# NivekNey/polars-matmul

Measured on AMD Instinct MI355X. Metric: cosine top-k queries/sec, higher is better.
Workload: dtype f32

## Files before the change

polars-matmul_amd/csrc/pmm_capi.hip:

```cpp
#include "pmm_internal.h"
#include "../../include/pmm.h"

#include <hip/hip_runtime.h>

#include <algorithm>
#include <atomic>
#include <cmath>
#include <cstdarg>
#include <cstdio>
#include <cstdlib>
#include <cstring>
#include <mutex>
#include <string>
#include <type_traits>
#include <vector>

using namespace pmm;

namespace {

constexpr const char *kVersion = "0.1.4+mi355x.r1";
constexpr size_t kMaterialiseBudget = size_t(2) << 30;

thread_local std::string t_err;
// ... 877 lines not shown
                               out_score, s));
  return PMM_OK;
}

int topk_f32_screened(const TopkRoute &r, const float *q, int64_t ldq, int64_t m, const float *c, int64_t ldc,
                      int64_t n, int64_t d, int64_t k, uint32_t index_base, uint32_t *out_idx, float *out_score,
                      char *w, hipStream_t s, int cus, const ScreenImage *img = nullptr,
                      const float *c_norms = nullptr) {
  const int metric = kMetricCosine;
  const ScreenPlan &sp = r.sp;
  const Plan &p = r.p;
  float *qn = (float *)(w + p.off_qn);
  const float *cn = img ? c_norms : (float *)(w + p.off_cn);
  uint16_t *qb = (uint16_t *)(w + sp.off_qb);
  const uint16_t *cb = img ? img->cb : (uint16_t *)(w + sp.off_cb);
  float *rel = (float *)(w + sp.off_rel), *eps = (float *)(w + sp.off_eps);
  unsigned *bad = (unsigned *)(w + sp.off_bad), *ovf = (unsigned *)(w + sp.off_ovf);
  unsigned *scal = (unsigned *)(w + sp.off_scal);
  int *rows = (int *)(w + sp.off_rows);
  HIP_TRY(hipMemsetAsync(w, 0, p.off_gthr + (size_t)m * 8, s));
  if (p.qb_full) HIP_TRY(hipMemsetAsync(w + p.off_cnt, 0, (size_t)m * p.S * 4, s));
  HIP_TRY(hipMemsetAsync(w + sp.off_ovf, 0, sp.off_rows - sp.off_ovf, s));
  if (img) {
    Timed t("norms_f32/prepare", s);
    HIP_TRY(launch_screen_prepare(q, m, d, ldq, qb, sp.dpb, qn, nullptr, rel, bad, nullptr, s));
    uint32_t bits;
    memcpy(&bits, &img->max_rel, 4);
    HIP_TRY(hipMemsetD32Async((hipDeviceptr_t)scal, (int)bits, 1, s));
  } else {
    Timed t("norms_f32/round", s);
    float *wcn = (float *)(w + p.off_cn), *crel = (float *)(w + sp.off_crel);
    HIP_TRY(launch_screen_prepare(q, m, d, ldq, qb, sp.dpb, qn, nullptr, rel, bad, nullptr, s));
    HIP_TRY(launch_screen_prepare(c, n, d, ldc, (uint16_t *)(w + sp.off_cb), sp.dpb, wcn, wcn + n, crel,
                                  (unsigned *)(crel + n), scal, s));
  }
  GemmF32Args a = fused_args(m, n, sp.dpb, k, metric, p, w);
  a.qb = qb;
  a.cb = cb;
  a.qn = qn;
  a.cn = cn;
  a.cpre = cn + n;
  a.ldq = sp.dpb;
  a.ldc = sp.dpb;
  set_bf16_knobs(a);
  const bool debug = getenv("PMM_SCREEN_DEBUG") != nullptr;
  a.eps = eps;
  a.ovf = ovf;
  {
    const int64_t ns = kSeedMaxNs;
    const int seed_env = getenv("PMM_BF16_SEED") ? atoi(getenv("PMM_BF16_SEED")) : 1;
    const bool seeded = seed_env && 4 * k <= ns && n >= 8 * ns && (size_t)m * ns * 4 <= p.off_qn - p.off_cand;
    Timed t("seed_bf16/screen", s);
    if (seeded) {
      float *sample = (float *)a.cand;
      HIP_TRY(launch_seed_bf16_ws(a, sample, (int)ns, s));
      HIP_TRY(launch_seed_select(sample, ns, (int)m, (int)ns, (int)k, metric, a.gthr, s));
    }
    HIP_TRY(launch_screen_prep(rel, scal, (int)m, (int)sp.dpb, eps, a.gthr, seeded ? 1 : 0, s));
  }
  {
    Timed t("gemm_f32_topk/screen", s);
    HIP_TRY(launch_gemm_bf16_ws(a, p.grid, s, true));
  }
  {
    Timed t("merge_topk/rescore", s);
    ScreenFinishArgs fa{};
    fa.q = q;
    fa.c = c;
    fa.ldq = ldq;
    fa.ldc = ldc;
    fa.qn = qn;
    fa.cn = cn;
    fa.eps = eps;
    fa.M = (int)m;
    fa.N = (int)n;
    fa.dp = (int)sp.dp;
    fa.S = p.S;
    fa.capg = p.capg;
    fa.k = (int)k;
    fa.cand = a.cand;
    fa.cnt = a.cnt;
    fa.gthr = a.gthr;
    fa.stat = debug ? scal + 4 : nullptr;
    HIP_TRY(launch_screen_rescore(fa, s));
  }
  {
    Timed t("merge_topk", s);
    HIP_TRY(launch_merge(merge_cand_args(a, p, index_base, out_idx, out_score), 0, s));
  }
  HIP_TRY(launch_zero_sign_f32(q, ldq, c, ldc, qn, cn, (int)m, n, (int)d, (int)k, metric, index_base, out_idx,
                               out_score, s));
  HIP_TRY(launch_screen_collect(ovf, bad, (int)m, scal + 2, rows, s));
  unsigned h[8] = {0, 0, 0, 0, 0, 0, 0, 0};
  HIP_TRY(hipMemcpyAsync(h, scal, 32, hipMemcpyDeviceToHost, s));
  HIP_TRY(hipStreamSynchronize(s));
  const bool whole = h[1] != 0 || (int64_t)h[2] * 8 > m + 8 * kScreenRerunRows;
  if (debug) {
    float rc;
    memcpy(&rc, &h[0], 4);
    fprintf(stderr,
            "[pmm screen] S=%d tps=%d qb_full=%d capg=%d ctrig=%d corpus_residual=%.6g corpus_unsafe=%u "
            "rerun_rows=%u overflowed=%u whole_call_f32=%d rescored=%u max_per_row=%u kept=%u m=%lld handle=%d\n",
            p.S, p.tps, p.qb_full, p.capg, p.ctrig, rc, h[1], h[2], h[3], whole ? 1 : 0, h[4], h[5], h[6],
            (long long)m, img ? 1 : 0);
  }
  if (whole) {
    const TopkRoute f = route_topk(m, n, d, k, metric, PMM_COMPUTE_F32, cus, false, false);
    return topk_f32_fused(f.p, q, ldq, m, c, ldc, n, d, k, metric, index_base, out_idx, out_score, w + sp.off_f32,
                          s, cus, c_norms, false);
  }
  for (int64_t r0 = 0; r0 < (int64_t)h[2]; r0 += sp.rr) {
    const int64_t nr = std::min<int64_t>(sp.rr, (int64_t)h[2] - r0);
    const TopkRoute f = route_topk(nr, n, d, k, metric, PMM_COMPUTE_F32, cus, false, false);
    const int rc = rerun_rows(q, ldq * 4, sp.dp * 4, rows + r0, nr, k, f.total, w + sp.off_gq, sp.total - sp.off_gq,
                              out_idx, out_score, s, "screen re-run",
                              [&](const char *gq, uint32_t *gi, float *gs, char *fw) {
                                return topk_f32_fused(f.p, (const float *)gq, sp.dp, nr, c, ldc, n, d, k, metric,
                                                      index_base, gi, gs, fw, s, cus, c_norms, false);
                              });
    if (rc) return rc;
  }
  return PMM_OK;
}

int topk_f32_unscreened(const TopkRoute &r, const float *q, int64_t ldq, int64_t m, const float *c, int64_t ldc,
                        int64_t n, int64_t d, int64_t k, int metric, uint32_t index_base, uint32_t *out_idx,
                        float *out_score, char *w, hipStream_t s, int cus, const float *c_norms, bool keep_gthr,
                        const float *c_pre = nullptr) {
  return r.fused ? topk_f32_fused(r.p, q, ldq, m, c, ldc, n, d, k, metric, index_base, out_idx, out_score, w, s, cus,
                                  c_norms, keep_gthr, c_pre)
                 : topk_f32_materialised(r.mp, q, ldq, m, c, ldc, n, d, k, metric, index_base, out_idx, out_score, w,
                                         s, cus, c_norms);
}

int topk_f32_device_impl(const TopkRoute &route, const float *q, int64_t ldq, int64_t m, const float *c, int64_t ldc,
                         int64_t n, int64_t d, int64_t k, int metric, uint32_t index_base, uint32_t *out_idx,
                         float *out_score, void *ws, size_t ws_bytes, hipStream_t s, int dev,
                         const float *c_norms = nullptr, bool keep_gthr = false,
                         const ScreenImage *img = nullptr, const float *c_pre = nullptr) {
  const int cus = g_dev[dev].cus;
  const int64_t dp = padded_dim(PMM_DTYPE_F32, d);
  TopkRoute plain;
  const TopkRoute *r = &route;
  if (route.kind == Route::kF32Screened &&
      ((c_norms != nullptr) != (img != nullptr) || route.sp.ext != (img != nullptr) || keep_gthr || ldq % 4 != 0 ||
       ldc % 4 != 0 || ldq < dp || ldc < dp || (((uintptr_t)q | (uintptr_t)c) & 15))) {
    plain = route_topk(m, n, d, k, metric, PMM_COMPUTE_F32, cus, false, false);
    r = &plain;
  }
  Workspace W;
  if (int rc = acquire_workspace(ws, ws_bytes, r->total, dev, s, W)) return rc;
  const int rc = r->kind == Route::kF32Screened
                     ? topk_f32_screened(*r, q, ldq, m, c, ldc, n, d, k, index_base, out_idx, out_score, W.w, s, cus,
                                         img, c_norms)
                     : topk_f32_unscreened(*r, q, ldq, m, c, ldc, n, d, k, metric, index_base, out_idx, out_score,
                                           W.w, s, cus, c_norms, keep_gthr, c_pre);
  return rc ? rc : W.done();
}

int topk_bf16_native(const Plan &p, const uint16_t *q, int64_t ldq, int64_t m, const uint16_t *c, int64_t ldc,
                     int64_t n, int64_t d, int64_t k, int metric, uint32_t index_base, uint32_t *out_idx,
                     float *out_score, char *w, hipStream_t s, const float *q_norms = nullptr,
                     const float *c_norms = nullptr) {
  const int64_t dp = padded_dim(PMM_DTYPE_BF16, d);
  const float *qn = q_norms ? q_norms : (const float *)(w + p.off_qn);
  const float *cn = c_norms ? c_norms : (const float *)(w + p.off_cn);
  HIP_TRY(hipMemsetAsync(w, 0, p.off_gthr + (size_t)m * 8, s));
  if (p.qb_full) HIP_TRY(hipMemsetAsync(w + p.off_cnt, 0, (size_t)m * p.S * 4, s));
  if (metric != kMetricDot && (!q_norms || !c_norms)) {
    const int sq = metric == kMetricEuclidean;
    Timed t("norms_bf16", s);
    if (!q_norms) HIP_TRY(launch_norms_bf16(q, m, d, ldq, sq, (float *)(w + p.off_qn), nullptr, s));
    if (!c_norms)
      HIP_TRY(launch_norms_bf16(c, n, d, ldc, sq, (float *)(w + p.off_cn), (float *)(w + p.off_cn) + n, s));
  }
  GemmF32Args a = fused_args(m, n, dp, k, metric, p, w);
  a.qb = q;
  a.cb = c;
  a.qn = qn;
  a.cn = cn;
  a.cpre = cn + n;
  a.ldq = ldq;
  a.ldc = ldc;
  set_bf16_knobs(a);
#ifdef PMM_LAB
  {
    static const int ablate = getenv("PMM_ABLATE") ? atoi(getenv("PMM_ABLATE")) : 0;
// ... 3731 lines not shown
```

polars-matmul_amd/csrc/pmm_internal.h:

```cpp
#pragma once
#include <hip/hip_runtime.h>
#include <stddef.h>
#include <stdint.h>

namespace pmm {

#ifdef PMM_LAB
#define PMM_ABL(x) (x)
#else
#define PMM_ABL(x) 0
#endif

constexpr int kMetricCosine = 0;
constexpr int kMetricDot = 1;
constexpr int kMetricEuclidean = 2;

constexpr int kFusedMaxK = 1024;
constexpr int kRowSelMaxP = 4096;

struct GemmF32Args {
  const float *q;
  const float *c;
  const uint16_t *qb;
  const uint16_t *cb;
// ... 175 lines not shown
  uint32_t *out_len;
};
hipError_t launch_maxsim_decode(const MaxsimDecodeArgs &a, hipStream_t s);
constexpr int kKmeansPiece = 256;
constexpr int kKmeansSortRows = 1024;
hipError_t launch_kmeans_labels(const uint32_t *oi, const float *os, int64_t n, uint32_t K, uint32_t *labels,
                                float *scores, bool have_prev, unsigned *changed, hipStream_t s);
struct KmeansOrder {
  const uint32_t *labels;
  int64_t n;
  uint32_t K;
  uint32_t *key[2], *val[2];
  uint32_t *hist, *base;
  uint32_t *bounds;
  uint32_t *pbase;
};
int64_t kmeans_sort_units(int64_t n);
int kmeans_sort_passes(uint32_t K);
int64_t kmeans_max_pieces(int64_t n, int64_t K);
hipError_t launch_kmeans_order(const KmeansOrder &a, hipStream_t s);
const uint32_t *kmeans_sorted_rows(const KmeansOrder &a);
struct KmeansUpdateArgs {
  const float *x;
  int64_t ldx;
  const float *cn;
  const uint32_t *rows, *bounds, *pbase;
  uint32_t K;
  int d, dp;
  int64_t max_pieces;
  double *psum;
  uint32_t *pcount;
  float *C;
};
hipError_t launch_kmeans_update(const KmeansUpdateArgs &a, hipStream_t s);
hipError_t launch_kmeans_finish(const KmeansUpdateArgs &a, hipStream_t s);
hipError_t launch_merge(const MergeArgs &a, int loader, hipStream_t s);
constexpr int kSeedMaxNs = 1024;
constexpr int kSeedDotsMaxD = 2048;
hipError_t launch_seeded_prologue(const float *q, int64_t ldq, int m, const float *c, int64_t ldc, int64_t n,
                                  int d, int dp, int ns, int k, int metric, float *qn, float *cn, bool corpus_norms,
                                  unsigned long long *gthr, void *z0, size_t z0_bytes, void *z1, size_t z1_bytes,
                                  hipStream_t s);
hipError_t launch_seed_select(const float *S, int64_t lds, int m, int ns, int k, int metric,
                              unsigned long long *gthr, hipStream_t s);
constexpr int kBf16BM = 128, kBf16BN = 128, kBf16NW = 4;
constexpr int kBf16MaxD = 768;
constexpr int kBf16DAlign = 128;
constexpr int kBf16MaxCapg = 1024;
hipError_t launch_gemm_bf16(const GemmF32Args &a, int grid, hipStream_t s);
size_t gemm_bf16_lds_bytes(int capg, int nst);
constexpr int kBf16WsBN = 64;
constexpr int kBf16WsMaxCapg = 512;
size_t gemm_bf16_ws_lds_bytes(int capg, int D);
hipError_t launch_gemm_bf16_ws(const GemmF32Args &a, int grid, hipStream_t s, bool screen = false);
hipError_t launch_seed_bf16_ws(const GemmF32Args &a, float *S, int ns, hipStream_t s);
constexpr int kBf16FfBM = 256, kBf16FfBN = 32;
size_t gemm_bf16_ff_lds_bytes(int D);
hipError_t launch_gemm_bf16_ff(const GemmF32Args &a, int grid, hipStream_t s);
hipError_t launch_ff_bucket(const GemmF32Args &a, unsigned *fb_count, int *fb_rows, hipStream_t s);
hipError_t launch_f32_to_bf16(const float *src, int64_t rows, int64_t d, int64_t lds, uint16_t *dst,
                              int64_t ldd, hipStream_t s);
hipError_t launch_round_norms_bf16(const float *src, int64_t rows, int64_t d, int64_t lds, uint16_t *dst,
                                   int64_t ldd, float *norm, float *inv_norm, float *sq, float *sq_factor,
                                   hipStream_t s);
hipError_t launch_bf16_to_f32(const uint16_t *src, int64_t rows, int64_t d, int64_t lds, float *dst, int64_t ldd,
                              hipStream_t s);
hipError_t launch_norms_bf16(const uint16_t *a, int64_t rows, int64_t d, int64_t ld, int squared,
                             float *out, float *inv, hipStream_t s);
size_t merge_lds_bytes_per_wave(int P);
hipError_t launch_screen_prepare(const float *src, int64_t rows, int64_t d, int64_t lds, uint16_t *dst, int64_t ldd,
                                 float *norm, float *inv_norm, float *rel, unsigned *bad, unsigned *scal,
                                 hipStream_t s);
hipError_t launch_screen_prep(const float *rel, const unsigned *scal, int m, int dp, float *eps,
                              unsigned long long *gthr, int seeded, hipStream_t s);
struct ScreenFinishArgs {
  const float *q, *c;
  int64_t ldq, ldc;
  const float *qn, *cn, *eps;
  int M, N, dp, S, capg, k;
  unsigned long long *cand;
  const unsigned *cnt;
  const unsigned long long *gthr;
  unsigned *stat;
};
hipError_t launch_screen_rescore(const ScreenFinishArgs &a, hipStream_t s);
hipError_t launch_screen_collect(const unsigned *ovf, const unsigned *bad, int m, unsigned *count, int *rows,
                                 hipStream_t s);
hipError_t launch_zero_sign_f32(const float *q, int64_t ldq, const float *c, int64_t ldc, const float *qn,
                                const float *cn, int m, int64_t n, int d, int k, int metric, uint32_t index_base,
                                const uint32_t *out_idx, float *out_score, hipStream_t s);
hipError_t launch_zero_sign_f64(const double *q, int64_t ldq, const double *c, int64_t ldc, const double *qn,
                                const double *cn, int m, int64_t n, int d, int k, int metric, uint32_t index_base,
                                const uint32_t *out_idx, double *out_score, hipStream_t s);
hipError_t launch_zero_sign_lists(const uint32_t *in_idx, const float *in_score, int lists, int k_in,
                                  int64_t row_stride, int64_t list_stride, int m, int k, const uint32_t *out_idx,
                                  float *out_score, hipStream_t s);
hipError_t launch_gather_rows(const void *src, int64_t ld_units, const int *rows, int r, int units, void *dst,
                              hipStream_t s);
hipError_t launch_scatter_lists(const uint32_t *oi, const float *os, const int *rows, int r, int k,
                                uint32_t *out_idx, float *out_score, hipStream_t s);
constexpr int kMaskBlockRows = 256 * 64;
hipError_t launch_mask_count(const unsigned long long *words, int shift, int64_t n, uint32_t *counts,
                             hipStream_t s);
hipError_t launch_mask_scan(const uint32_t *counts, int64_t nblk, uint32_t *bases, hipStream_t s);
hipError_t launch_mask_write(const unsigned long long *words, int shift, int64_t n, const uint32_t *bases,
                             uint32_t *out, hipStream_t s);
hipError_t launch_subset_gather(const void *src, const uint32_t *ids, int64_t s, int units, void *dst,
                                const void *aux_src, void *aux_dst, int na, int aux_bytes, int64_t n_src,
                                int flag_arr, unsigned *any, hipStream_t st);
hipError_t launch_remap_index(uint32_t *idx, int64_t count, const uint32_t *map, int64_t s, hipStream_t st);
constexpr int kGroupedMaxK = 128;
constexpr int kGroupedMaxDp = 1024;
constexpr int kGroupedRows = 16;
struct GroupedUnit {
  uint32_t c0, ng, q0, mq;
};
struct GroupedArgs {
  const float *q;
  const float *c;
  const float *qn, *cn;
  int64_t ldq, ldc;
  int dp, k;
  const GroupedUnit *units;
  uint32_t *out_idx;
  float *out_score;
};
size_t grouped_lds_bytes(int dp);
hipError_t launch_grouped_topk_f32(const GroupedArgs &a, int units, int metric, hipStream_t s);
hipError_t launch_grouped_pad(const uint32_t *si, const void *ss, int rows, int kg, int k, uint32_t *di, void *ds,
                              bool f64, hipStream_t s);
hipError_t launch_grouped_scatter(const uint32_t *gi, const void *gs, const uint32_t *qrow, const uint32_t *glen,
                                  int64_t rows, int k, const uint32_t *map, uint32_t n, uint32_t *out_idx,
                                  void *out_score, uint32_t *out_len, bool f64, hipStream_t s);
hipError_t launch_gemm_f64_store(const double *q, int64_t ldq, const double *c, int64_t ldc,
                                 const double *qn, const double *cn, int M, int N, int D,
                                 int metric, int store_metric, double *out, int64_t ldo,
                                 hipStream_t s);
hipError_t launch_rowselect(const RowSelArgs &a, hipStream_t s);
struct Ent;
struct F64TopkArgs {
  const double *q;
  const double *c;
  const double *qn, *cn;
  int64_t ldq, ldc;
  int M, D;
  int col0, ncol;
  int metric;
  const unsigned long long *tkey;
  const uint32_t *tidx;
  unsigned *cnt;
  Ent *cand;
  int cap;
  int accept_all;
};
struct F64SelArgs {
  Ent *cand;
  unsigned *cnt;
  int cap, M, k, P;
  int mode;
  unsigned long long *tkey;
  uint32_t *tidx;
  int metric;
  uint32_t index_base;
  uint32_t *out_idx;
  double *out_score;
  unsigned *overflow;
// ... 75 lines not shown
```

polars-matmul_amd/csrc/pmm_kernels.hip:

```cpp
#include "pmm_device.h"

#include <algorithm>

#include <hip/hip_runtime.h>
#include <math.h>
#include <stdint.h>

#include <type_traits>

namespace pmm {

hipError_t launch_norms_f32(const float *a, int64_t rows, int64_t d, int64_t ld, int squared,
                            float *out, float *inv, hipStream_t s) {
  if (rows <= 0) return hipSuccess;
  const int64_t threads = rows * 8;
  const unsigned grid = (unsigned)((threads + 255) / 256);
  norms_kernel<float><<<grid, 256, 0, s>>>(a, rows, d, ld, squared, out, inv);
  return hipGetLastError();
}
hipError_t launch_norms_pair_f32(const float *q, int64_t m, int64_t ldq, float *qout, const float *c,
                                 int64_t n, int64_t ldc, float *cout, float *cinv, int64_t d, int squared,
                                 hipStream_t s, void *zero, size_t zero_bytes) {
  const unsigned gq = (unsigned)((m * 8 + 255) / 256), gc = (unsigned)((n * 8 + 255) / 256);
  if (zero_bytes % 16 != 0 || ((uintptr_t)zero & 15)) return hipErrorInvalidValue;
// ... 1936 lines not shown
  const int64_t t = (int64_t)blockIdx.x * blockDim.x + threadIdx.x;
  const int64_t half = (int64_t)P2 >> 1;
  if (t >= (int64_t)rows * half) return;
  const int r = (int)(t / half), i = (int)(t % half);
  const int x0 = ((i & ~(stride - 1)) << 1) | (i & (stride - 1));
  const int x1 = x0 + stride;
  Ent *base = keys + (int64_t)r * P2;
  const Ent a = base[x0], b = base[x1];
  const bool desc = (x0 & size) == 0;
  if (desc ? ent_better(b, a) : ent_better(a, b)) {
    base[x0] = b;
    base[x1] = a;
  }
}
template <typename T>
__global__ void rowsort_extract(const Ent *__restrict__ keys, int rows, int P2, int k, int metric,
                                uint32_t index_base, uint32_t *__restrict__ out_idx,
                                T *__restrict__ out_score) {
  const int64_t t = (int64_t)blockIdx.x * blockDim.x + threadIdx.x;
  if (t >= (int64_t)rows * k) return;
  const int r = (int)(t / k), j = (int)(t % k);
  const Ent e = keys[(int64_t)r * P2 + j];
  out_idx[t] = e.idx + index_base;
  out_score[t] = key_score<T>(e.key, metric);
}

hipError_t launch_rowsort_global(const void *scores, int64_t lds, int rows, int N, int is_f64,
                                 int metric, void *keys_ws, int P2, int k, uint32_t index_base,
                                 uint32_t *out_idx, void *out_score, hipStream_t s) {
  if (rows <= 0) return hipSuccess;
  Ent *keys = (Ent *)keys_ws;
  const int64_t tot = (int64_t)rows * P2;
  const unsigned gb = (unsigned)((tot + 255) / 256);
  if (is_f64) rowsort_build<double><<<gb, 256, 0, s>>>((const double *)scores, lds, rows, N, P2, metric, keys);
  else rowsort_build<float><<<gb, 256, 0, s>>>((const float *)scores, lds, rows, N, P2, metric, keys);
  const unsigned gs = (unsigned)((tot / 2 + 255) / 256);
  for (int size = 2; size <= P2; size <<= 1)
    for (int stride = size >> 1; stride > 0; stride >>= 1)
      rowsort_step<<<gs, 256, 0, s>>>(keys, rows, P2, size, stride);
  const int64_t tk = (int64_t)rows * k;
  const unsigned ge = (unsigned)((tk + 255) / 256);
  if (is_f64) rowsort_extract<double><<<ge, 256, 0, s>>>(keys, rows, P2, k, metric, index_base, out_idx, (double *)out_score);
  else rowsort_extract<float><<<ge, 256, 0, s>>>(keys, rows, P2, k, metric, index_base, out_idx, (float *)out_score);
  return hipGetLastError();
}

__global__ __launch_bounds__(256) void screen_prep_kernel(const float *__restrict__ rel,
                                                          const unsigned *__restrict__ scal, int m, int dp,
                                                          float *__restrict__ eps, u64 *gthr, int seeded) {
  const int row = (int)(blockIdx.x * blockDim.x + threadIdx.x);
  if (row >= m) return;
  const float e = screen_eps(rel[row], __uint_as_float(scal[0]), dp);
  eps[row] = e;
  if (seeded) gthr[row] = screen_lower(gthr[row], e);
}
hipError_t launch_screen_prep(const float *rel, const unsigned *scal, int m, int dp, float *eps,
                              unsigned long long *gthr, int seeded, hipStream_t s) {
  if (m <= 0) return hipSuccess;
  screen_prep_kernel<<<(unsigned)((m + 255) / 256), 256, 0, s>>>(rel, scal, m, dp, eps, gthr, seeded);
  return hipGetLastError();
}

constexpr int kRescoreList = 512;

template <typename F>
__device__ __forceinline__ void rescore_each_entry(const ScreenFinishArgs &a, u64 *base, const unsigned *segs,
                                                   int nseg, F &&f) {
  const int tid = threadIdx.x, nt = blockDim.x;
  for (int t = 0; t < nseg; t++) {
    const unsigned e = segs[t];
    const int n = (int)(e & 1023u);
    u64 *seg = base + (int64_t)(e >> 10) * a.capg;
    for (int i0 = tid; i0 < n; i0 += 4 * nt) {
      u64 x[4];
#pragma unroll
      for (int j = 0; j < 4; j++) x[j] = i0 + j * nt < n ? seg[i0 + j * nt] : 0ull;
#pragma unroll
      for (int j = 0; j < 4; j++)
        if (i0 + j * nt < n) f(seg + i0 + j * nt, x[j]);
    }
  }
}

__global__ __launch_bounds__(256, 8) void screen_rescore_kernel(ScreenFinishArgs a) {
  extern __shared__ __attribute__((aligned(16))) char smem[];
  __shared__ __attribute__((aligned(16))) unsigned hist[256];
  __shared__ unsigned list[kRescoreList];
  __shared__ unsigned res[4], ln, emin;
  float *qs = (float *)smem;
  unsigned *segs = (unsigned *)(qs + a.dp);
  const int tid = threadIdx.x, nt = blockDim.x;
  const int row = (int)blockIdx.x;
  const float *qr = a.q + (int64_t)row * a.ldq;
  for (int i = 4 * tid; i < a.dp; i += 4 * nt) *(f32x4 *)(qs + i) = *(const f32x4 *)(qr + i);
  for (int i = tid; i < 256; i += nt) hist[i] = 0u;
  if (tid == 0) emin = ~0u, ln = 0u;
  __syncthreads();
  for (int s = tid; s < a.S; s += nt) {
    const unsigned n = min(a.cnt[(int64_t)row * a.S + s], (unsigned)a.capg);
    if (n) segs[atomicAdd(&ln, 1u)] = ((unsigned)s << 10) | n;
  }
  __syncthreads();
  const int nseg = (int)ln;
  const float qv = a.qn[row];
  const float eps = a.eps[row];
  const u64 T = screen_lower(a.gthr[row], eps);
  const u64 T1 = T ? T : 1ull;
  u64 *base = a.cand + (int64_t)row * a.S * a.capg;

  auto live = [&](u64 x) __attribute__((always_inline)) -> bool {
    return x >= T1 && ~(uint32_t)x < (uint32_t)a.N;
  };
  u64 P = 0ull;
  unsigned n_r = 0u, need = (unsigned)a.k;
  for (int shift = 56; shift >= 0; shift -= 8) {
    rescore_each_entry(a, base, segs, nseg, [&](u64 *, u64 x) __attribute__((always_inline)) {
      if (live(x) && (shift == 56 || ((x ^ P) >> (shift + 8)) == 0ull))
        atomicAdd(&hist[(unsigned)(x >> shift) & 255u], 1u);
    });
    __syncthreads();
    if (tid < 64) {
      const uint4 h = ((const uint4 *)hist)[tid];
      ((uint4 *)hist)[tid] = make_uint4(0u, 0u, 0u, 0u);
      const unsigned own = h.x + h.y + h.z + h.w;
      unsigned suf = own;
#pragma unroll
      for (int o = 1; o < 64; o <<= 1) {
        const unsigned t = __shfl_down(suf, o);
        if (tid + o < 64) suf += t;
      }
      if (tid == 0) {
        res[0] = res[1] = res[2] = 0u;
        if (shift == 56) res[3] = suf;
      }
      unsigned above = suf - own;
      if (above < need && suf >= need) {
        unsigned b = 3u, in_bin = h.w;
        if (above + in_bin < need) above += in_bin, in_bin = h.z, b = 2u;
        if (above + in_bin < need) above += in_bin, in_bin = h.y, b = 1u;
        if (above + in_bin < need) above += in_bin, in_bin = h.x, b = 0u;
        res[0] = 4u * (unsigned)tid + b;
        res[1] = need - above;
        res[2] = in_bin;
      }
    }
    __syncthreads();
    P |= (u64)res[0] << shift;
    need = res[1];
    if (shift == 56) n_r = res[3];
    if (res[2] == need) break;
  }
  const int max_rounds = (int)(((int64_t)a.S * a.capg + kRescoreList - 1) / kRescoreList) + 1;
  unsigned done = 0u;
  for (int ph = n_r > (unsigned)a.k ? 1 : 2; ph <= 2; ph++) {
    const bool last = ph == 2;
    u64 thr = P;
    if (last) {
      __syncthreads();
      const u64 E = screen_lower((u64)emin << 32, eps);
      thr = E > T1 ? E : T1;
    }
    for (int r = 0; r < max_rounds; r++) {
      __syncthreads();
      if (tid == 0) ln = 0u;
      __syncthreads();
      rescore_each_entry(a, base, segs, nseg, [&](u64 *p, u64 x) __attribute__((always_inline)) {
        if (x == 0ull) return;
        const uint32_t lw = (uint32_t)x;
        if (!(lw & 0x80000000u)) return;
        if (x < thr || !live(x)) {
          if (last) *p = 0ull;
          return;
        }
        const unsigned pos = atomicAdd(&ln, 1u);
        if (pos < (unsigned)kRescoreList) list[pos] = (unsigned)(p - base);
      });
      __syncthreads();
      const unsigned n = ln;
      const bool more = n > (unsigned)kRescoreList;
      const int cnt = more ? kRescoreList : (int)n;
      for (int t = tid; t < cnt; t += nt) {
        u64 *p = base + list[t];
        const uint32_t col = ~(uint32_t)*p;
        const float *cr = a.c + (int64_t)col * a.ldc;
        float acc = 0.0f;
        for (int k0 = 0; k0 < a.dp; k0 += 32) {
          f32x4 v[8];
#pragma unroll
          for (int j = 0; j < 8; j++) v[j] = *(const f32x4 *)(cr + k0 + 4 * j);
#pragma unroll
          for (int j = 0; j < 8; j++) {
            const f32x4 q4 = *(const f32x4 *)(qs + k0 + 4 * j);
            acc = fmaf(q4[0], v[j][0], acc);
            acc = fmaf(q4[1], v[j][1], acc);
            acc = fmaf(q4[2], v[j][2], acc);
            acc = fmaf(q4[3], v[j][3], acc);
          }
        }
        const uint32_t key = okey32(exact_score<kMetricCosine>(acc, qv, a.cn[col]));
        if (!last) atomicMin(&emin, key);
        *p = ((u64)key << 32) | (u64)col;
        done++;
      }
      if (!more) break;
    }
  }
  __syncthreads();
  rescore_each_entry(a, base, segs, nseg, [&](u64 *p, u64 x) __attribute__((always_inline)) {
    if (x != 0ull && !((uint32_t)x & 0x80000000u)) *p = (x & 0xFFFFFFFF00000000ull) | (u64)(~(uint32_t)x);
  });
  if (a.stat) {
    __syncthreads();
    if (tid == 0) ln = 0u;
    __syncthreads();
    atomicAdd(&ln, done);
    __syncthreads();
    if (tid == 0) {
      atomicAdd(a.stat, ln);
      atomicMax(a.stat + 1, ln);
      atomicAdd(a.stat + 2, n_r);
    }
  }
}
hipError_t launch_screen_rescore(const ScreenFinishArgs &a, hipStream_t s) {
  if (a.M <= 0) return hipSuccess;
  if (a.dp % 32 != 0 || a.dp > 4096 || a.ldq % 4 != 0 || a.ldc % 4 != 0 || a.ldq < a.dp || a.ldc < a.dp ||
      (((uintptr_t)a.q | (uintptr_t)a.c) & 15) || a.k < 1 || a.k > kRescoreList || a.capg > 1023 ||
      ((int64_t)a.dp + a.S) * 4 > 64 * 1024)
    return hipErrorInvalidValue;
  int nt = 64;
  if (const char *e = getenv("PMM_RESCORE_BLOCK")) {
    const int v = atoi(e);
    if (v == 64 || v == 128 || v == 256) nt = v;
  }
  screen_rescore_kernel<<<(unsigned)a.M, nt, ((size_t)a.dp + a.S) * 4, s>>>(a);
  return hipGetLastError();
}

__device__ __forceinline__ bool is_pos_zero(float v) { return __float_as_uint(v) == 0u; }
__device__ __forceinline__ bool is_pos_zero(double v) { return __double_as_longlong(v) == 0ll; }
__device__ __forceinline__ float fma_chain_step(float a, float b, float c) { return fmaf(a, b, c); }
__device__ __forceinline__ double fma_chain_step(double a, double b, double c) { return __fma_rn(a, b, c); }
__device__ __forceinline__ float cosine_of(float dot, float qv, float cv) {
  return exact_score<kMetricCosine>(dot, qv, cv);
}
__device__ __forceinline__ double cosine_of(double dot, double qv, double cv) {
  return exact_score_f64<kMetricCosine>(dot, qv, cv);
}
template <typename T>
__global__ __launch_bounds__(256) void zero_sign_kernel(const T *__restrict__ q, int64_t ldq,
                                                        const T *__restrict__ c, int64_t ldc,
                                                        const T *__restrict__ qn, const T *__restrict__ cn,
                                                        int m, int64_t n, int d, int k, int metric,
                                                        uint32_t index_base, const uint32_t *__restrict__ out_idx,
                                                        T *__restrict__ out_score) {
  const int64_t t = (int64_t)blockIdx.x * blockDim.x + threadIdx.x;
  if (t >= (int64_t)m * k) return;
  if (!is_pos_zero(out_score[t])) return;
  const uint32_t id = out_idx ? out_idx[t] : (uint32_t)(t % k) + index_base;
  if (id == 0xFFFFFFFFu) return;
  const int64_t col = (int64_t)(uint32_t)(id - index_base);
  if (col >= n) return;
  const int row = (int)(t / k);
  const T *qr = q + (int64_t)row * ldq, *cr = c + col * ldc;
  T acc = (T)0;
  for (int i = 0; i < d; i++) acc = fma_chain_step(qr[i], cr[i], acc);
  const T sc = metric == kMetricDot ? acc : cosine_of(acc, qn[row], cn[col]);
  if (sc == (T)0) out_score[t] = sc;
}
hipError_t launch_zero_sign_f32(const float *q, int64_t ldq, const float *c, int64_t ldc, const float *qn,
                                const float *cn, int m, int64_t n, int d, int k, int metric, uint32_t index_base,
                                const uint32_t *out_idx, float *out_score, hipStream_t s) {
  if (m <= 0 || k <= 0 || metric == kMetricEuclidean) return hipSuccess;
  zero_sign_kernel<float><<<(unsigned)(((int64_t)m * k + 255) / 256), 256, 0, s>>>(
      q, ldq, c, ldc, qn, cn, m, n, d, k, metric, index_base, out_idx, out_score);
  return hipGetLastError();
}
hipError_t launch_zero_sign_f64(const double *q, int64_t ldq, const double *c, int64_t ldc, const double *qn,
                                const double *cn, int m, int64_t n, int d, int k, int metric, uint32_t index_base,
                                const uint32_t *out_idx, double *out_score, hipStream_t s) {
  if (m <= 0 || k <= 0 || metric == kMetricEuclidean) return hipSuccess;
  zero_sign_kernel<double><<<(unsigned)(((int64_t)m * k + 255) / 256), 256, 0, s>>>(
      q, ldq, c, ldc, qn, cn, m, n, d, k, metric, index_base, out_idx, out_score);
  return hipGetLastError();
}

__global__ __launch_bounds__(256) void zero_sign_lists_kernel(const uint32_t *__restrict__ in_idx,
                                                              const float *__restrict__ in_score, int lists,
                                                              int k_in, int64_t row_stride, int64_t list_stride,
                                                              int m, int k, const uint32_t *__restrict__ out_idx,
                                                              float *__restrict__ out_score) {
  const int64_t t = (int64_t)blockIdx.x * blockDim.x + threadIdx.x;
  if (t >= (int64_t)m * k) return;
  if (__float_as_uint(out_score[t]) != 0u) return;
  const uint32_t id = out_idx[t];
  if (id == 0xFFFFFFFFu) return;
  const int64_t row = t / k;
  for (int g = 0; g < lists; g++) {
    const int64_t base = (int64_t)g * list_stride + row * row_stride;
    for (int j = 0; j < k_in; j++) {
      if (in_idx[base + j] != id) continue;
      const float sc = in_score[base + j];
      if (sc == 0.0f) out_score[t] = sc;
      return;
    }
  }
}
hipError_t launch_zero_sign_lists(const uint32_t *in_idx, const float *in_score, int lists, int k_in,
                                  int64_t row_stride, int64_t list_stride, int m, int k, const uint32_t *out_idx,
                                  float *out_score, hipStream_t s) {
  if (m <= 0 || k <= 0 || lists <= 0) return hipSuccess;
  zero_sign_lists_kernel<<<(unsigned)(((int64_t)m * k + 255) / 256), 256, 0, s>>>(
      in_idx, in_score, lists, k_in, row_stride, list_stride, m, k, out_idx, out_score);
  return hipGetLastError();
}

__global__ __launch_bounds__(256) void screen_collect_kernel(const unsigned *__restrict__ ovf,
// ... 51 lines not shown
```

Measured before the change: 614,500.

## Stage rescore candidates in LDS with fallback to global-memory kernel

Result: no change. 618,900, median of 6 (+0.7%).

```diff
diff --git a/polars-matmul_amd/csrc/pmm_capi.hip b/polars-matmul_amd/csrc/pmm_capi.hip
--- a/polars-matmul_amd/csrc/pmm_capi.hip
+++ b/polars-matmul_amd/csrc/pmm_capi.hip
@@ -983,6 +983,8 @@
     fa.cnt = a.cnt;
     fa.gthr = a.gthr;
     fa.stat = debug ? scal + 4 : nullptr;
+    fa.fb_rows = rows;
+    fa.fb_count = scal + 7;
     HIP_TRY(launch_screen_rescore(fa, s));
   }
   {
@@ -1001,9 +1003,10 @@
     memcpy(&rc, &h[0], 4);
     fprintf(stderr,
             "[pmm screen] S=%d tps=%d qb_full=%d capg=%d ctrig=%d corpus_residual=%.6g corpus_unsafe=%u "
-            "rerun_rows=%u overflowed=%u whole_call_f32=%d rescored=%u max_per_row=%u kept=%u m=%lld handle=%d\n",
+            "rerun_rows=%u overflowed=%u whole_call_f32=%d rescored=%u max_per_row=%u kept=%u m=%lld handle=%d "
+            "fallback_rows=%u\n",
             p.S, p.tps, p.qb_full, p.capg, p.ctrig, rc, h[1], h[2], h[3], whole ? 1 : 0, h[4], h[5], h[6],
-            (long long)m, img ? 1 : 0);
+            (long long)m, img ? 1 : 0, h[7]);
   }
   if (whole) {
     const TopkRoute f = route_topk(m, n, d, k, metric, PMM_COMPUTE_F32, cus, false, false);
diff --git a/polars-matmul_amd/csrc/pmm_internal.h b/polars-matmul_amd/csrc/pmm_internal.h
--- a/polars-matmul_amd/csrc/pmm_internal.h
+++ b/polars-matmul_amd/csrc/pmm_internal.h
@@ -281,6 +281,8 @@
   const unsigned *cnt;
   const unsigned long long *gthr;
   unsigned *stat;
+  int *fb_rows;
+  unsigned *fb_count;
 };
 hipError_t launch_screen_rescore(const ScreenFinishArgs &a, hipStream_t s);
 hipError_t launch_screen_collect(const unsigned *ovf, const unsigned *bad, int m, unsigned *count, int *rows,
diff --git a/polars-matmul_amd/csrc/pmm_kernels.hip b/polars-matmul_amd/csrc/pmm_kernels.hip
--- a/polars-matmul_amd/csrc/pmm_kernels.hip
+++ b/polars-matmul_amd/csrc/pmm_kernels.hip
@@ -2042,6 +2042,52 @@
   }
 }
 
+__device__ __forceinline__ void rescore_pick_bin(unsigned *hist, unsigned *res, int tid, unsigned need, bool first) {
+  const uint4 h = ((const uint4 *)hist)[tid];
+  ((uint4 *)hist)[tid] = make_uint4(0u, 0u, 0u, 0u);
+  const unsigned own = h.x + h.y + h.z + h.w;
+  unsigned suf = own;
+#pragma unroll
+  for (int o = 1; o < 64; o <<= 1) {
+    const unsigned t = __shfl_down(suf, o);
+    if (tid + o < 64) suf += t;
+  }
+  if (tid == 0) {
+    res[0] = res[1] = res[2] = 0u;
+    if (first) res[3] = suf;
+  }
+  unsigned above = suf - own;
+  if (above < need && suf >= need) {
+    unsigned b = 3u, in_bin = h.w;
+    if (above + in_bin < need) above += in_bin, in_bin = h.z, b = 2u;
+    if (above + in_bin < need) above += in_bin, in_bin = h.y, b = 1u;
+    if (above + in_bin < need) above += in_bin, in_bin = h.x, b = 0u;
+    res[0] = 4u * (unsigned)tid + b;
+    res[1] = need - above;
+    res[2] = in_bin;
+  }
+}
+
+__device__ __forceinline__ uint32_t rescore_gather_key(const ScreenFinishArgs &a, const float *qs, float qv,
+                                                       uint32_t col) {
+  const float *cr = a.c + (int64_t)col * a.ldc;
+  float acc = 0.0f;
+  for (int k0 = 0; k0 < a.dp; k0 += 32) {
+    f32x4 v[8];
+#pragma unroll
+    for (int j = 0; j < 8; j++) v[j] = *(const f32x4 *)(cr + k0 + 4 * j);
+#pragma unroll
+    for (int j = 0; j < 8; j++) {
+      const f32x4 q4 = *(const f32x4 *)(qs + k0 + 4 * j);
+      acc = fmaf(q4[0], v[j][0], acc);
+      acc = fmaf(q4[1], v[j][1], acc);
+      acc = fmaf(q4[2], v[j][2], acc);
+      acc = fmaf(q4[3], v[j][3], acc);
+    }
+  }
+  return okey32(exact_score<kMetricCosine>(acc, qv, a.cn[col]));
+}
+
 __global__ __launch_bounds__(256, 8) void screen_rescore_kernel(ScreenFinishArgs a) {
   extern __shared__ __attribute__((aligned(16))) char smem[];
   __shared__ __attribute__((aligned(16))) unsigned hist[256];
@@ -2050,7 +2096,11 @@
   float *qs = (float *)smem;
   unsigned *segs = (unsigned *)(qs + a.dp);
   const int tid = threadIdx.x, nt = blockDim.x;
-  const int row = (int)blockIdx.x;
+  int row = (int)blockIdx.x;
+  if (a.fb_rows) {
+    if (blockIdx.x >= *a.fb_count) return;
+    row = a.fb_rows[blockIdx.x];
+  }
   const float *qr = a.q + (int64_t)row * a.ldq;
   for (int i = 4 * tid; i < a.dp; i += 4 * nt) *(f32x4 *)(qs + i) = *(const f32x4 *)(qr + i);
   for (int i = tid; i < 256; i += nt) hist[i] = 0u;
@@ -2079,31 +2129,7 @@
         atomicAdd(&hist[(unsigned)(x >> shift) & 255u], 1u);
     });
     __syncthreads();
-    if (tid < 64) {
-      const uint4 h = ((const uint4 *)hist)[tid];
-      ((uint4 *)hist)[tid] = make_uint4(0u, 0u, 0u, 0u);
-      const unsigned own = h.x + h.y + h.z + h.w;
-      unsigned suf = own;
-#pragma unroll
-      for (int o = 1; o < 64; o <<= 1) {
-        const unsigned t = __shfl_down(suf, o);
-        if (tid + o < 64) suf += t;
-      }
-      if (tid == 0) {
-        res[0] = res[1] = res[2] = 0u;
-        if (shift == 56) res[3] = suf;
-      }
-      unsigned above = suf - own;
-      if (above < need && suf >= need) {
-        unsigned b = 3u, in_bin = h.w;
-        if (above + in_bin < need) above += in_bin, in_bin = h.z, b = 2u;
-        if (above + in_bin < need) above += in_bin, in_bin = h.y, b = 1u;
-        if (above + in_bin < need) above += in_bin, in_bin = h.x, b = 0u;
-        res[0] = 4u * (unsigned)tid + b;
-        res[1] = need - above;
-        res[2] = in_bin;
-      }
-    }
+    if (tid < 64) rescore_pick_bin(hist, res, tid, need, shift == 56);
     __syncthreads();
     P |= (u64)res[0] << shift;
     need = res[1];
@@ -2142,22 +2168,7 @@
       for (int t = tid; t < cnt; t += nt) {
         u64 *p = base + list[t];
         const uint32_t col = ~(uint32_t)*p;
-        const float *cr = a.c + (int64_t)col * a.ldc;
-        float acc = 0.0f;
-        for (int k0 = 0; k0 < a.dp; k0 += 32) {
-          f32x4 v[8];
-#pragma unroll
-          for (int j = 0; j < 8; j++) v[j] = *(const f32x4 *)(cr + k0 + 4 * j);
-#pragma unroll
-          for (int j = 0; j < 8; j++) {
-            const f32x4 q4 = *(const f32x4 *)(qs + k0 + 4 * j);
-            acc = fmaf(q4[0], v[j][0], acc);
-            acc = fmaf(q4[1], v[j][1], acc);
-            acc = fmaf(q4[2], v[j][2], acc);
-            acc = fmaf(q4[3], v[j][3], acc);
-          }
-        }
-        const uint32_t key = okey32(exact_score<kMetricCosine>(acc, qv, a.cn[col]));
+        const uint32_t key = rescore_gather_key(a, qs, qv, col);
         if (!last) atomicMin(&emin, key);
         *p = ((u64)key << 32) | (u64)col;
         done++;
@@ -2182,6 +2193,163 @@
     }
   }
 }
+
+#ifndef PMM_RESCORE_KSTAGE
+#define PMM_RESCORE_KSTAGE 512
+#endif
+constexpr int kRescoreStage = PMM_RESCORE_KSTAGE;
+static_assert(kRescoreStage >= 1 && kRescoreStage <= 4096, "the list holds 16-bit stage slots; LDS");
+
+__global__ __launch_bounds__(64, 4) void screen_rescore_staged_kernel(ScreenFinishArgs a, int stage) {
+  extern __shared__ __attribute__((aligned(16))) char smem[];
+  __shared__ __attribute__((aligned(16))) unsigned hist[256];
+  __shared__ unsigned res[4], emin;
+  u64 *st = (u64 *)smem;
+  float *qs = (float *)(st + ((stage + 1) & ~1));
+  unsigned *segs = (unsigned *)(qs + a.dp);
+  unsigned *sbeg = segs + a.S;
+  unsigned short *list = (unsigned short *)hist;
+  const int tid = threadIdx.x;
+  const int row = (int)blockIdx.x;
+  const u64 below = (1ull << tid) - 1ull;
+  const float *qr = a.q + (int64_t)row * a.ldq;
+  for (int i = 4 * tid; i < a.dp; i += 256) *(f32x4 *)(qs + i) = *(const f32x4 *)(qr + i);
+  for (int i = tid; i < 256; i += 64) hist[i] = 0u;
+  if (tid == 0) emin = ~0u;
+  int nseg = 0;
+  unsigned total = 0u;
+  for (int s0 = 0; s0 < a.S; s0 += 64) {
+    const int s = s0 + tid;
+    const unsigned n = s < a.S ? min(a.cnt[(int64_t)row * a.S + s], (unsigned)a.capg) : 0u;
+    unsigned inc = n;
+#pragma unroll
+    for (int o = 1; o < 64; o <<= 1) {
+      const unsigned t = __shfl_up(inc, o);
+      if (tid >= o) inc += t;
+    }
+    const u64 m = __ballot(n != 0u);
+    if (n) {
+      const int pos = nseg + __popcll(m & below);
+      segs[pos] = ((unsigned)s << 10) | n;
+      sbeg[pos] = total + inc - n;
+    }
+    total += __shfl(inc, 63);
+    nseg += __popcll(m);
+  }
+  if (total > (unsigned)stage) {
+    if (tid == 0) a.fb_rows[atomicAdd(a.fb_count, 1u)] = row;
+    return;
+  }
+  __syncthreads();
+  const float qv = a.qn[row];
+  const float eps = a.eps[row];
+  const u64 T = screen_lower(a.gthr[row], eps);
+  const u64 T1 = T ? T : 1ull;
+  u64 *base = a.cand + (int64_t)row * a.S * a.capg;
+  int lg = 0;
+  while (lg < 31 && (1 << lg) < nseg) lg++;
+  auto slot = [&](unsigned j) __attribute__((always_inline)) -> u64 * {
+    int lo = 0, hi = nseg - 1;
+    for (int it = 0; it < lg; it++) {
+      const int mid = (lo + hi + 1) >> 1;
+      if (sbeg[mid] <= j) lo = mid;
+      else hi = mid - 1;
+    }
+    const unsigned e = segs[lo];
+    const unsigned i = min(j - sbeg[lo], (e & 1023u) - 1u);
+    return base + (int64_t)(e >> 10) * a.capg + i;
+  };
+  for (unsigned j0 = 0; j0 < total; j0 += 512u) {
+    u64 x[8];
+#pragma unroll
+    for (int u = 0; u < 8; u++) x[u] = *slot(min(j0 + 64u * u + tid, total - 1u));
+#pragma unroll
+    for (int u = 0; u < 8; u++)
+      if (j0 + 64u * u + tid < total) st[j0 + 64u * u + tid] = x[u];
+  }
+  __syncthreads();
+
+  auto live = [&](u64 x) __attribute__((always_inline)) -> bool {
+    return x >= T1 && ~(uint32_t)x < (uint32_t)a.N;
+  };
+  u64 P = 0ull;
+  unsigned n_r = 0u, need = (unsigned)a.k;
+  for (int shift = 56; shift >= 0; shift -= 8) {
+    for (unsigned j = tid; j < total; j += 64u) {
+      const u64 x = st[j];
+      if (live(x) && (shift == 56 || ((x ^ P) >> (shift + 8)) == 0ull))
+        atomicAdd(&hist[(unsigned)(x >> shift) & 255u], 1u);
+    }
+    __syncthreads();
+    rescore_pick_bin(hist, res, tid, need, shift == 56);
+    __syncthreads();
+    P |= (u64)res[0] << shift;
+    need = res[1];
+    if (shift == 56) n_r = res[3];
+    if (res[2] == need) break;
+  }
+  const int max_rounds = (int)(total / (unsigned)kRescoreList) + 1;
+  unsigned done = 0u;
+  for (int ph = n_r > (unsigned)a.k ? 1 : 2; ph <= 2; ph++) {
+    const bool last = ph == 2;
+    u64 thr = P;
+    if (last) {
+      __syncthreads();
+      const u64 E = screen_lower((u64)emin << 32, eps);
+      thr = E > T1 ? E : T1;
+    }
+    for (int r = 0; r < max_rounds; r++) {
+      __syncthreads();
+      unsigned n = 0u;
+      for (unsigned j0 = 0; j0 < total; j0 += 64u) {
+        const unsigned j = j0 + tid;
+        bool keep = false;
+        if (j < total) {
+          const u64 x = st[j];
+          if (x != 0ull && ((uint32_t)x & 0x80000000u)) {
+            if (x < thr || !live(x)) {
+              if (last) st[j] = 0ull;
+            } else {
+              keep = true;
+            }
+          }
+        }
+        const u64 m = __ballot(keep);
+        const unsigned pos = n + (unsigned)__popcll(m & below);
+        if (keep && pos < (unsigned)kRescoreList) list[pos] = (unsigned short)j;
+        n += (unsigned)__popcll(m);
+      }
+      __syncthreads();
+      const bool more = n > (unsigned)kRescoreList;
+      const int cnt = more ? kRescoreList : (int)n;
+      for (int t = tid; t < cnt; t += 64) {
+        const unsigned j = list[t];
+        const uint32_t col = ~(uint32_t)st[j];
+        const uint32_t key = rescore_gather_key(a, qs, qv, col);
+        if (!last) atomicMin(&emin, key);
+        st[j] = ((u64)key << 32) | (u64)col;
+        done++;
+      }
+      if (!more) break;
+    }
+  }
+  __syncthreads();
+  for (unsigned j = tid; j < total; j += 64u) {
+    const u64 x = st[j];
+    const bool scored = x != 0ull && !((uint32_t)x & 0x80000000u);
+    *slot(j) = scored ? (x & 0xFFFFFFFF00000000ull) | (u64)(~(uint32_t)x) : x;
+  }
+  if (a.stat) {
+#pragma unroll
+    for (int o = 32; o > 0; o >>= 1) done += __shfl_xor(done, o);
+    if (tid == 0) {
+      atomicAdd(a.stat, done);
+      atomicMax(a.stat + 1, done);
+      atomicAdd(a.stat + 2, n_r);
+    }
+  }
+}
+
 hipError_t launch_screen_rescore(const ScreenFinishArgs &a, hipStream_t s) {
   if (a.M <= 0) return hipSuccess;
   if (a.dp % 32 != 0 || a.dp > 4096 || a.ldq % 4 != 0 || a.ldc % 4 != 0 || a.ldq < a.dp || a.ldc < a.dp ||
@@ -2193,6 +2361,20 @@
     const int v = atoi(e);
     if (v == 64 || v == 128 || v == 256) nt = v;
   }
+  int stage = kRescoreStage;
+  if (const char *e = getenv("PMM_RESCORE_STAGE")) {
+    const int v = atoi(e);
+    if (v >= 0 && v <= kRescoreStage) stage = v;
+  }
+  const size_t staged_lds = (size_t)((stage + 1) & ~1) * 8 + (size_t)a.dp * 4 + (size_t)a.S * 8;
+  if (stage == 0 || !a.fb_rows || !a.fb_count || staged_lds > 60 * 1024) {
+    ScreenFinishArgs all = a;
+    all.fb_rows = nullptr;
+    all.fb_count = nullptr;
+    screen_rescore_kernel<<<(unsigned)a.M, nt, ((size_t)a.dp + a.S) * 4, s>>>(all);
+    return hipGetLastError();
+  }
+  screen_rescore_staged_kernel<<<(unsigned)a.M, 64, staged_lds, s>>>(a, stage);
   screen_rescore_kernel<<<(unsigned)a.M, nt, ((size_t)a.dp + a.S) * 4, s>>>(a);
   return hipGetLastError();
 }
```
